# dangut/RGBiD-SLAM

Measured on AMD Instinct MI355X. Metric: aligned RGB-D frames/sec @640x480, 3-level pyr; achieved HBM GB/s vs roofline, higher is better.
Workload: dtype f32

## Files before the change

include/rgbid_batched.h:

```cpp
#ifndef RGBID_BATCHED_H_
#define RGBID_BATCHED_H_

#include "rgbid.h"

#ifdef __cplusplus
extern "C" {
#endif

typedef struct rgbid_imgb {
  void*  data;
  size_t step;
  size_t lane_stride;
  int    rows, cols;
} rgbid_imgb;

typedef struct rgbid_sys_params {
  float sigma_depthinv, sigma_int, bias_depthinv, bias_int, nu_depthinv, nu_int;
  int mestimator, weighting;
  int student_nu;
  int nu_int_from_max;
} rgbid_sys_params;

enum {
  RGBID_WM_AUTO = -1,
// ... 15 lines not shown
                            const rgbid_imgb* dst_iD, const rgbid_imgb* dst_I, const float* R_proj, const float* t_proj,
                            int numerics, float* ms);

int rgbid_lattice_pack_batched(rgbid_ctx*, int lanes, const rgbid_imgb* W0, const rgbid_imgb* I0, int min_nsamples, float* out_dev,
                               size_t out_lane_stride, float* ms);
int rgbid_lattice_residuals_batched(rgbid_ctx*, int lanes, const rgbid_imgb* Wcur, const rgbid_imgb* W0, const rgbid_imgb* Icur,
                                    const rgbid_imgb* I0, const float* R_proj, const float* t_proj, int min_nsamples, int numerics,
                                    const float* kf_lat_dev, size_t kf_lat_lane_stride, float* res_dev, size_t res_lane_stride,
                                    float* ms);
int rgbid_lattice_residuals_raw_batched(rgbid_ctx*, int lanes, const rgbid_imgb* Wcur, const rgbid_imgb* W0, const rgbid_imgb* Icur,
                                        const rgbid_imgb* I0, const float* R_proj, const float* t_proj, int min_nsamples, int numerics,
                                        const float* kf_lat_dev, size_t kf_lat_lane_stride, float* res_dev, size_t res_lane_stride,
                                        const rgbid_imgb* depth_u16, const rgbid_imgb* rgb_u8x3, float factor_depth, const int* lane_on_dev,
                                        float* ms);
int rgbid_frame_px_batched(rgbid_ctx*, int lanes, const rgbid_imgb* depth_u16, const rgbid_imgb* rgb_u8x3, const rgbid_imgb* depthinv,
                           const rgbid_imgb* intensity_pair, const rgbid_imgb* intensity_single, float factor_depth, float* ms);
typedef struct rgbid_scale_pair { float bias_depthinv, sigma_depthinv, nu_depthinv, bias_int, sigma_int, nu_int; } rgbid_scale_pair;
int rgbid_sigma_pair_batched(rgbid_ctx*, int lanes, const float* res_dev, size_t res_lane_stride, int n, int mestimator,
                             rgbid_scale_pair* out, float* ms);
int rgbid_sigma_pair_maps_batched(rgbid_ctx*, int lanes, const rgbid_imgb* W1, const rgbid_imgb* W0, const rgbid_imgb* I1, const rgbid_imgb* I0,
                                  int min_nsamples, int mestimator, rgbid_scale_pair* out, float* ms);

int rgbid_fuse_frame_batched(rgbid_ctx*, int lanes, const rgbid_imgb* cur_depthinv, const rgbid_imgb* kf_depthinv,
                             const rgbid_imgb* kf_weight, const rgbid_imgb* warped_weight, const float* R_proj, const float* t_proj,
                             int numerics, float* ms);
int rgbid_kf_maps_batched(rgbid_ctx*, int lanes, rgbid_intr intr, const rgbid_imgb* depthinv, const rgbid_imgb* vmap,
                          const rgbid_imgb* nmap, float* ms);
int rgbid_visibility_pair_batched(rgbid_ctx*, int lanes, const rgbid_imgb* a, const rgbid_imgb* b, const float* R_ab, const float* t_ab,
                                  const float* R_ba, const float* t_ba, int numerics, unsigned int* counts, float* ms);

int rgbid_prep_frame_batched(rgbid_ctx*, int lanes, const rgbid_imgb* depth_u16, const rgbid_imgb* rgb_u8x3, const rgbid_imgb* depthinv,
                             const rgbid_imgb* intensity, const rgbid_imgb* r, const rgbid_imgb* g, const rgbid_imgb* b,
                             float factor_depth, float* ms);
int rgbid_pyr_down_batched(rgbid_ctx*, int lanes, const rgbid_imgb* src, const rgbid_imgb* dst, float* ms);
int rgbid_compute_gradient_batched(rgbid_ctx*, int lanes, const rgbid_imgb* src, const rgbid_imgb* dst_hor, const rgbid_imgb* dst_vert,
                                   float* ms);
int rgbid_gradient_keep_batched(rgbid_ctx*, int lanes, const rgbid_imgb* src, const rgbid_imgb* dst_hor, const rgbid_imgb* dst_vert,
                                const rgbid_imgb* keep, float* ms);
int rgbid_bilateral_filter_batched(rgbid_ctx*, int lanes, const rgbid_imgb* src, const rgbid_imgb* dst, float sigma_floatmap,
                                   int numerics, float* ms);
int rgbid_pyr_down_pair_batched(rgbid_ctx*, int lanes, const rgbid_imgb* src0, const rgbid_imgb* dst0, const rgbid_imgb* src1,
                                const rgbid_imgb* dst1, float* ms);
int rgbid_gradient_pair_batched(rgbid_ctx*, int lanes, const rgbid_imgb* src0, const rgbid_imgb* dst_hor0, const rgbid_imgb* dst_vert0,
                                const rgbid_imgb* src1, const rgbid_imgb* dst_hor1, const rgbid_imgb* dst_vert1, float* ms);
int rgbid_gradient_keep_pair_batched(rgbid_ctx*, int lanes, const rgbid_imgb* src0, const rgbid_imgb* dst_hor0, const rgbid_imgb* dst_vert0,
                                     const rgbid_imgb* keep0, const rgbid_imgb* src1, const rgbid_imgb* dst_hor1,
                                     const rgbid_imgb* dst_vert1, const rgbid_imgb* keep1, float* ms);
int rgbid_bilateral_pair_batched(rgbid_ctx*, int lanes, const rgbid_imgb* src0, const rgbid_imgb* dst0, float sigma_floatmap0,
                                 const rgbid_imgb* src1, const rgbid_imgb* dst1, float sigma_floatmap1, int numerics, float* ms);

#ifdef __cplusplus
}
#endif
#endif
```

rgbid-slam_amd/csrc/c_api_batched.hip:

```cpp
#include "../../include/rgbid_batched.h"
#include "hip_host.h"
#include "kernels.h"

#include <cstring>
#include <vector>

using namespace rgbid;

namespace {

const LaneMask ALL{nullptr, 0};

inline bool ok_b(const rgbid_imgb* i, int lanes, size_t elem = 4) {
  const size_t align = elem == 3 ? 1 : elem;
  return i && i->data && lanes >= 1 && lanes <= 65535 && i->rows > 0 && i->cols > 0 && i->step >= (size_t)i->cols * elem && i->step % align == 0 &&
         ((uintptr_t)i->data) % align == 0 && i->rows < (1 << 24) && i->step < ((size_t)1 << 24) && (unsigned long long)i->rows * i->step < (1ull << 32) &&
         (lanes == 1 || (i->lane_stride >= (size_t)i->rows * i->step && i->lane_stride % align == 0));
}
inline bool same_b(const rgbid_imgb* a, const rgbid_imgb* b) { return a->rows == b->rows && a->cols == b->cols; }
inline ImgB BB(const rgbid_imgb* i, int lanes) { return ImgB{i->data, i->step, lanes == 1 ? 0 : i->lane_stride, i->rows, i->cols}; }
inline bool numerics_ok(int n) { return n == RGBID_NUMERICS_EXACT || n == RGBID_NUMERICS_FAST; }
inline bool al16(const rgbid_imgb* a, int lanes) { return (a->step & 15) == 0 && (lanes == 1 || (a->lane_stride & 15) == 0) && (((uintptr_t)a->data) & 15) == 0; }

struct Call {
// ... 305 lines not shown
  const size_t off_ab = 0, off_ba = up256(sizeof(WarpParams) * lanes), off_cnt = off_ba + up256(sizeof(WarpParams) * lanes);
  int e = ctx_reserve_lane(c, off_cnt + sizeof(unsigned int) * 4 * lanes);
  if (e) return e;
  if ((e = staging_free(c))) return e;
  if ((e = stage_warps(c, lanes, R_ab, t_ab, off_ab))) return e;
  if ((e = stage_warps(c, lanes, R_ba, t_ba, off_ba))) return e;
  if ((e = staging_sent(c))) return e;
  unsigned int* cnt = reinterpret_cast<unsigned int*>((char*)c->lane_dev + off_cnt);
  RGBID_HIP(hipMemsetAsync(cnt, 0, sizeof(unsigned int) * 4 * lanes, c->stream));
  Call call(c, ms);
  launch_visibility_pair(c->stream, lanes, BB(a, lanes), BB(b, lanes), reinterpret_cast<const WarpParams*>((char*)c->lane_dev + off_ab),
                         reinterpret_cast<const WarpParams*>((char*)c->lane_dev + off_ba), cnt, cnt + 2 * lanes, ALL, numerics == RGBID_NUMERICS_FAST);
  e = call.finish(cnt, sizeof(unsigned int) * 4 * lanes, off_cnt);
  if (e) return e;
  const unsigned int* h = reinterpret_cast<const unsigned int*>((char*)c->lane_host + off_cnt);
  for (int l = 0; l < lanes; ++l) {
    counts[4 * l + 0] = h[2 * l + 0]; counts[4 * l + 1] = h[2 * l + 1];
    counts[4 * l + 2] = h[2 * lanes + 2 * l + 0]; counts[4 * l + 3] = h[2 * lanes + 2 * l + 1];
  }
  return RGBID_OK;
}

int rgbid_prep_frame_batched(rgbid_ctx* c, int lanes, const rgbid_imgb* depth, const rgbid_imgb* rgb, const rgbid_imgb* iD, const rgbid_imgb* I, const rgbid_imgb* r,
                             const rgbid_imgb* g, const rgbid_imgb* b, float factor_depth, float* ms) {
  const rgbid_imgb* all[7] = {depth, rgb, iD, I, r, g, b};
  if (!c || lanes < 1 || !(factor_depth == factor_depth) || factor_depth == 0.f) return RGBID_E_INVALID;
  for (int i = 0; i < 7; ++i) if (!ok_b(all[i], lanes, i == 0 ? 2 : i == 1 ? 3 : 4) || !same_b(all[i], iD)) return RGBID_E_INVALID;
  hipSetDevice(c->device);
  Call call(c, ms);
  launch_prep_frame(c->stream, lanes, BB(depth, lanes), BB(rgb, lanes), BB(iD, lanes), BB(I, lanes), BB(r, lanes), BB(g, lanes), BB(b, lanes), factor_depth, ALL);
  return call.finish();
}

int rgbid_pyr_down_batched(rgbid_ctx* c, int lanes, const rgbid_imgb* src, const rgbid_imgb* dst, float* ms) {
  if (!c || lanes < 1 || !ok_b(src, lanes) || !ok_b(dst, lanes) || dst->rows != src->rows / 2 || dst->cols != src->cols / 2) return RGBID_E_INVALID;
  hipSetDevice(c->device);
  Call call(c, ms);
  launch_pyr_down(c->stream, lanes, BB(src, lanes), BB(dst, lanes), ALL);
  return call.finish();
}

int rgbid_compute_gradient_batched(rgbid_ctx* c, int lanes, const rgbid_imgb* src, const rgbid_imgb* gx, const rgbid_imgb* gy, float* ms) {
  if (!c || lanes < 1 || !ok_b(src, lanes) || !ok_b(gx, lanes) || !ok_b(gy, lanes) || !same_b(src, gx) || !same_b(src, gy)) return RGBID_E_INVALID;
  hipSetDevice(c->device);
  Call call(c, ms);
  launch_gradient(c->stream, lanes, BB(src, lanes), BB(gx, lanes), BB(gy, lanes), ALL);
  return call.finish();
}

int rgbid_gradient_keep_batched(rgbid_ctx* c, int lanes, const rgbid_imgb* src, const rgbid_imgb* gx, const rgbid_imgb* gy, const rgbid_imgb* keep, float* ms) {
  if (!c || lanes < 1 || !ok_b(src, lanes) || !ok_b(gx, lanes) || !ok_b(gy, lanes) || !ok_b(keep, lanes) || !same_b(src, gx) || !same_b(src, gy) || !same_b(src, keep) ||
      src->data == keep->data)
    return RGBID_E_INVALID;
  hipSetDevice(c->device);
  Call call(c, ms);
  const bool launched = launch_gradient_keep(c->stream, lanes, BB(src, lanes), BB(gx, lanes), BB(gy, lanes), BB(keep, lanes), ALL);
  const int r = call.finish();
  return launched ? r : RGBID_E_INVALID;
}

int rgbid_bilateral_filter_batched(rgbid_ctx* c, int lanes, const rgbid_imgb* src, const rgbid_imgb* dst, float sigma_floatmap, int numerics, float* ms) {
  if (!c || lanes < 1 || !ok_b(src, lanes) || !ok_b(dst, lanes) || !same_b(src, dst) || src->data == dst->data || !numerics_ok(numerics) ||
      !(sigma_floatmap > 0.f))
    return RGBID_E_INVALID;
  hipSetDevice(c->device);
  Call call(c, ms);
// ... 54 lines not shown
```

rgbid-slam_amd/csrc/engine.hip:

```cpp
#include "../../include/rgbid_engine.h"
#include "hip_host.h"
#include "kernels.h"
#include "../../include/rgbid/se3.h"
#include "engine_device.h"
#include "step_plan.h"
#include "sigma_device.h"

#include <algorithm>
#include <cassert>
#include <cstdio>
#include <cstdlib>
#include <cstring>
#include <new>
#include <vector>

#pragma clang fp contract(off)

using namespace rgbid;
using namespace rgbid::eng;

constexpr int MAXL = 8;

namespace {

// ... 131 lines not shown
  __shared__ WarpParams next_warp;
  __shared__ int update_ok;
  reduce_partials<256>(partials, nblk, lane, tid, sm, sums);
  if (tid == 0) {
    LaneState& s = st[lane];
    GnUpdate u;
    gn_update(sums, pin ? s.alt_R : s.cur_R, pin ? s.alt_t : s.cur_t, u);
    if (!u.failed) set_warp_from_pose(c, level, u.R, u.t, next_warp);
    update_ok = u.failed ? 0 : 1;
    if (blockIdx.x == 0) gn_commit(u, s, pin ? s.cur_R : s.alt_R, pin ? s.cur_t : s.alt_t, f, wp, &next_warp, c, level, lane);
  }
  __syncthreads();
  if (!update_ok) return;
  const int i = blockIdx.x * 256 + tid;
  if (i >= n) return;
  FusedLatticeGetter g{Wcur, Icur, W0, I0, next_warp, lane, stride, interp_mode, fast};
  const int ly = i / lcols, lx = i - ly * lcols;
  float rd, ri;
  if (kf_lat) {
    const float* k = kf_lat + (size_t)lane * kf_lat_lane_stride;
    g.both_given(ly, lx, k[i], k[n + i], rd, ri);
  } else {
    g.both(ly, lx, rd, ri);
  }
  float* r = res + (size_t)lane * res_lane_stride;
  r[i] = rd; r[n + i] = ri;
}
inline int update_prologue_max_lanes() {
  const char* e = getenv("RGBID_ENGINE_UPDATE_PROLOGUE_LANES");
  return e ? atoi(e) : 8;
}
inline bool lattice_raw_enabled() {
  const char* e = getenv("RGBID_ENGINE_LATTICE_RAW");
  return !(e && atoi(e) == 0);
}
inline int scalar_block_threads(int B) { return B > 256 ? 64 : 256; }

__global__ void k_level_begin(Flags f, int B) {
  int lane = blockIdx.x * blockDim.x + threadIdx.x;
  if (lane < B) f.lvl[lane] = f.gn[lane];
}
__global__ __launch_bounds__(64) RGBID_SCALAR_KERNEL void k_chi_decide(LaneState* st, Flags f, const float* chi_out, WarpParams* wp, StepCfg c, int iter, int after_level, int B) {
  int lane = blockIdx.x * blockDim.x + threadIdx.x;
  if (lane >= B || !f.lvl[lane]) return;
  LaneState& s = st[lane];
  const float RMSE = sqrtf(chi_out[3 * lane + 0]) / sqrtf(chi_out[3 * lane + 2]);
  if (iter != 1 && RMSE > s.rmse_prev) {
    double d[3], tmp[3];
    for (int i = 0; i < 3; ++i) d[i] = s.cur_t[i] - s.inc_t[i];
    se3::m3_mulv(s.inc_inv_R, d, tmp);
    for (int i = 0; i < 3; ++i) s.cur_t[i] = tmp[i];
    se3::m3_mul(s.inc_inv_R, s.cur_R, s.cur_R);
    f.lvl[lane] = 0;
    set_warp_from_pose(c, after_level, s.cur_R, s.cur_t, wp[lane]);
    return;
  }
  s.rmse_prev = RMSE;
}

template <int NT>
__global__ __launch_bounds__(NT) RGBID_SCALAR_KERNEL void k_frame_finish(const double* partials, int nblk, LaneState* st, Flags f, const SysParams* sp,
                                                      WarpParams* vis_ab, WarpParams* vis_ba, WarpParams* ivis_ab, WarpParams* ivis_ba,
                                                      rgbid_pose_record* rec, StepCfg c) {
  int lane = blockIdx.x;
  if (!f.track[lane]) return;
  __shared__ double sm[8][32];
// ... 398 lines not shown
  Ledger led;
  auto fast_at = [&](int level) {
    return c.fast_numerics != 0 && gn_fast_supported(e->iD_kf[level], e->I_kf[level], e->gxD[level], e->gyD[level], e->gxI[level], e->gyI[level], e->I_curr[level]);
  };
  auto warp_pair = [&](int l, LaneMask m) {
    if (!(fast_at(l) && launch_warp_pair_fast(s, B, e->iD_curr[l], e->I_curr[l], e->iD_kf[l], e->wiD[l], e->wI[l], nullptr, e->wp, c.interp_mode, m)))
      launch_warp_pair(s, B, e->iD_curr[l], e->I_curr[l], e->iD_kf[l], e->wiD[l], e->wI[l], e->wp, c.interp_mode, m);
    led.add(1, 0, 20 * npx(e->iD_kf[l]));
  };
  auto chi_lattice = [&](int l, LaneMask m, double bytes) {
    int n, lr, lc, st;
    lattice_geometry(e->wI[l].rows, e->wI[l].cols, 9999999, &n, &lr, &lc, &st);
    launch_error_lattice(s, B, e->wI[l], e->I_kf[l], e->res_I, res_stride, lr, lc, st, m);
    launch_error_lattice(s, B, e->wiD[l], e->iD_kf[l], e->res_D, res_stride, lr, lc, st, m);
    launch_chi_square(s, B, e->res_I, e->res_D, res_stride, n, 5.f, 0.0025f, c.mestimator, e->chi_out, m);
    led.add(3, 0, bytes);
  };
  auto kf_maps = [&](LaneMask m, int bucket, double fallback_bytes) {
    const int n = enqueue_kf_maps(e, s, m);
    led.add(n, bucket, n == 1 ? 28 * N0 : fallback_bytes);
  };
  auto system_events = [&](int level) {
    if (!(e->prof_on && level == 0 && e->prof_used + 2 <= (int)e->prof_ev.size())) return;
    set_system_kernel_events(e->prof_ev[e->prof_used], e->prof_ev[e->prof_used + 1]);
    e->prof_used += 2;
  };
  auto per_lane = [&](auto* k64, auto* k256, auto... args) {
    const int nt = scalar_block_threads(B);
    hipLaunchKernelGGL(nt == 64 ? k64 : k256, dim3(B), dim3(nt), 0, s, args...);
    led.add(1);
  };
  const LaneMask fed = M(e->active_dev);
  const bool custom = c.custom_registration != 0;
  launch_prep_frame(s, B, e->cur_depth, e->cur_rgb, custom ? e->iD_dist : e->iD_curr[0], custom ? e->I_dist : e->I_curr[0], e->r_curr, e->g_curr, e->b_curr, c.factor_depth, fed);
  led.add(1, 0, 25 * N0);
  if (custom) {
    const IntrK kc{c.fx, c.fy, c.cx, c.cy, c.rgb_dist[0], c.rgb_dist[1], c.rgb_dist[2], c.rgb_dist[3], c.rgb_dist[4]};
    const IntrK kd{c.depth_intr.fx, c.depth_intr.fy, c.depth_intr.cx, c.depth_intr.cy, c.depth_intr.k1, c.depth_intr.k2, c.depth_intr.k3, c.depth_intr.k4, c.depth_intr.k5};
    DepthDistP dp;
    dp.c1 = c.depth_dist.c1; dp.c0 = c.depth_dist.c0; dp.xshift = c.depth_dist.xshift; dp.yshift = c.depth_dist.yshift;
    for (int i = 0; i < 9; ++i) { dp.q0[i] = c.depth_dist.q0[i]; dp.q1[i] = c.depth_dist.q1[i]; }
    launch_undistort(s, B, e->I_dist, e->I_curr[0], kc, true, c.interp_mode, fed);
    led.add(1, 0, 12 * N0);
    launch_depthinv_correction(s, B, e->iD_dist, e->iD_corr, kd, dp, fed);
    led.add(1, 0, 8 * N0);
    launch_undistort(s, B, e->iD_corr, e->iD_prereg, kd, false, 0, fed);
    led.add(1, 0, 8 * N0);
    launch_register_depthinv(s, B, e->iD_prereg, e->reg_f, e->reg_i, e->iD_curr[0], c.dRc_proj, c.t_dc_proj, c.cRd_proj, fed);
    led.add(4, 0, (9 * 4 + 8 + 9 * 8 + 8) * N0);
  }
  for (int i = 1; i < L; ++i) {
    launch_pyr_down2(s, B, e->I_curr[i - 1], e->I_curr[i], e->iD_curr[i - 1], e->iD_curr[i], fed);
    led.add(1, 0, 2 * (4 * npx(e->I_curr[i - 1]) + 4 * npx(e->I_curr[i])));
  }
  hipLaunchKernelGGL(k_step_begin, dim3(gb), dim3(tb), 0, s, e->state, f, e->wp, e->sp, sc, B, e->counts, e->sched.start_sys_level, e->sched.start_sys_cov);
  led.add(1);
  if (!first) {
    const bool chi_stop = c.termination == RGBID_CHI_SQUARED, warp_first = c.warping == RGBID_WARP_FIRST, pdf = c.sigma_estimator == RGBID_SIGMA_PDF;
    const LaneMask LV = M(f.lvl), GN = M(f.gn);
    assert(!(c.fused_gn && (warp_first || chi_stop)));
    const bool prologue_plan = c.fused_gn && pdf && e->lat_res && B <= update_prologue_max_lanes();
    const RawFrame raw0{e->cur_depth, e->cur_rgb, c.factor_depth};
    const bool lattice_raw = lattice_raw_enabled() && !custom && !prologue_plan && fast_at(0) && lattice_raw_supported(raw0, e->iD_kf[0], B);
    struct { bool on; int nblk, sys_level, sys_cov; } pend = {false, 0, -1, 0};
    int pose_in_alt = 0;
    int nblk;
    for (const GnIter& g : e->sched.iters) {
      const int level = g.level;
      if (chi_stop && g.it == 0) { hipLaunchKernelGGL(k_level_begin, dim3(gb), dim3(tb), 0, s, f, B); led.add(1); }
      const double nl = npx(e->iD_kf[level]);
      const double ns = pdf ? (double)lattice_samples(e->iD_kf[level].rows, e->iD_kf[level].cols, c.nsamples) : 0.0;
      if (c.fused_gn) {
        if (pdf) {
          if (pend.on) {
            int n_, lr_, lc_, st_;
            lattice_geometry(e->iD_kf[level].rows, e->iD_kf[level].cols, c.nsamples, &n_, &lr_, &lc_, &st_);
            const size_t kls = 2 * e->lat_cap;
            hipLaunchKernelGGL(k_lattice_after_update, dim3(div_up(n_, 256), B), dim3(256), 0, s, e->iD_curr[level], e->iD_kf[level], e->I_curr[level], e->I_kf[level], c.interp_mode,
                               n_, lc_, st_, e->lat_res, 2 * e->lat_cap, kls >= 2 * (size_t)n_ ? e->lat_kf[level] : nullptr, kls, fast_at(level) ? 1 : 0,
                               e->partials, pend.nblk, e->state, f, e->wp, sc, level, e->sp, pend.sys_level, pend.sys_cov, pose_in_alt);
            launch_sigma_pair_arrays(s, B, e->lat_res, 2 * e->lat_cap, n_, e->sp, c.mestimator, LV);
            pose_in_alt ^= 1; pend.on = false;
          } else {
            launch_sigma_pair_fused(s, B, e->iD_curr[level], e->iD_kf[level], e->I_curr[level], e->I_kf[level], e->wp, c.interp_mode, c.nsamples,
// ... 508 lines not shown
```

rgbid-slam_amd/csrc/kernels.h:

```cpp
#pragma once
#include "common.h"

namespace rgbid {

struct SysParams {
  float fx, fy, cx, cy;
  float sigma_d, sigma_i, bias_d, bias_i, nu_d, nu_i;
  int mestimator, weighting, student_nu;
  int nu_i_max;
};
struct SigmaIO { float bias, sigma, nu; };
struct IntrP { float fx, fy, cx, cy; };
struct LightP { float x, y, z; };
struct IntrK { float fx, fy, cx, cy, k1, k2, k3, k4, k5; };
struct DepthDistP { float c1, c0, q0[9], q1[9]; int xshift, yshift; };

enum { SYS_TERMS = 27 };
static constexpr float TH_HUBER = 1.345f, TH_TUKEY = 4.685f, STUDENT_DOF = 5.f;

void launch_undistort(hipStream_t s, int B, ImgB src, ImgB dst, IntrK k, bool linear, int interp_mode, LaneMask m);
void launch_depthinv_correction(hipStream_t s, int B, ImgB src, ImgB dst, IntrK k, DepthDistP dp, LaneMask m);
void launch_register_depthinv(hipStream_t s, int B, ImgB src, ImgB inter_f, ImgB inter_i, ImgB dst, const float dRc_proj[9], const float t_dc_proj[3],
                              const float cRd_proj[9], LaneMask m);

void launch_depth_to_invdepth(hipStream_t s, int B, ImgB src_u16, ImgB dst, float factor_depth, LaneMask m);
void launch_intensity(hipStream_t s, int B, ImgB rgb, ImgB dst, LaneMask m);
void launch_depth_to_float(hipStream_t s, int B, ImgB src_u16, ImgB dst, LaneMask m);
void launch_float_to_rgb(hipStream_t s, int B, ImgB src, ImgB dst_rgb, LaneMask m);
void launch_warp_pair(hipStream_t s, int B, ImgB src_iD, ImgB src_I, ImgB grid, ImgB dst_iD, ImgB dst_I, const WarpParams* lane_params, int interp_mode, LaneMask m,
                      const WarpParams* host_p = nullptr);
bool launch_warp_pair_fast(hipStream_t s, int B, ImgB src_iD, ImgB src_I, ImgB grid, ImgB dst_iD, ImgB dst_I, const WarpParams* host_p, const WarpParams* lane_params,
                           int interp_mode, LaneMask m);
void launch_selftest_cvt_flr(hipStream_t s, unsigned long long* mismatches_dev, unsigned stride);
void launch_nmap_cross(hipStream_t s, int B, ImgB vmap, ImgB nmap, LaneMask m);
void launch_integrate_warped_rgb(hipStream_t s, int B, ImgB warped, ImgB r, ImgB g, ImgB b, ImgB wweight, ImgB kf, ImgB colors, ImgB kfw, LaneMask m);
void launch_decompose_rgb(hipStream_t s, int B, ImgB rgb, ImgB r, ImgB g, ImgB b, LaneMask m);
void launch_gradient(hipStream_t s, int B, ImgB src, ImgB gx, ImgB gy, LaneMask m);
bool launch_gradient_keep(hipStream_t s, int B, ImgB src, ImgB gx, ImgB gy, ImgB keep, LaneMask m);
void launch_prep_frame(hipStream_t s, int B, ImgB depth_u16, ImgB rgb, ImgB iD, ImgB I, ImgB r, ImgB g, ImgB b, float factor_depth, LaneMask m);
void launch_copy_bytes(hipStream_t s, int B, ImgB src, ImgB dst, int elem_size, LaneMask m);
void launch_fill(hipStream_t s, int B, ImgB dst, int elem_size, uint32_t bits, LaneMask m);
void launch_pyr_down(hipStream_t s, int B, ImgB src, ImgB dst, LaneMask m);
void launch_pyr_down2(hipStream_t s, int B, ImgB src0, ImgB dst0, ImgB src1, ImgB dst1, LaneMask m);
void launch_gradient2(hipStream_t s, int B, ImgB src0, ImgB gx0, ImgB gy0, ImgB src1, ImgB gx1, ImgB gy1, LaneMask m);
bool launch_gradient_keep2(hipStream_t s, int B, ImgB src0, ImgB gx0, ImgB gy0, ImgB keep0, ImgB src1, ImgB gx1, ImgB gy1, ImgB keep1, LaneMask m);
void launch_bilateral2(hipStream_t s, int B, ImgB src0, ImgB dst0, float sigma0, ImgB src1, ImgB dst1, float sigma1, LaneMask m, bool fast = false);
void launch_lattice_pack_levels(hipStream_t s, int B, int n_levels, const ImgB* W0, const ImgB* I0, int min_nsamples, float* const* out, size_t out_lane_stride, LaneMask m);
void launch_visibility_pair2(hipStream_t s, int B, ImgB a, ImgB b0, const WarpParams* p_ab0, const WarpParams* p_ba0, unsigned int* counts_ab0, unsigned int* counts_ba0,
                             ImgB b1, const WarpParams* p_ab1, const WarpParams* p_ba1, unsigned int* counts_ab1, unsigned int* counts_ba1, LaneMask m, bool fast);
void launch_bilateral(hipStream_t s, int B, ImgB src, ImgB dst, float sigma_floatmap, LaneMask m, bool fast = false);
bool div_const_verified(float c);
void launch_selftest_div_const(hipStream_t s, float c, unsigned long long* mismatches_dev);

void launch_warp_invdepth(hipStream_t s, int B, ImgB src, ImgB grid, ImgB dst, const WarpParams* host_p, const WarpParams* lane_p, LaneMask m);
void launch_warp_intensity(hipStream_t s, int B, ImgB src, ImgB grid, ImgB dst, const WarpParams* host_p, const WarpParams* lane_p, int interp_mode, LaneMask m);
void launch_warp_invdepth_weighted(hipStream_t s, int B, ImgB src, ImgB grid, ImgB dst, ImgB weight, const WarpParams* host_p, const WarpParams* lane_p, LaneMask m);
void launch_integrate_warped(hipStream_t s, int B, ImgB warped, ImgB wweight, ImgB kf, ImgB kfweight, LaneMask m);
void launch_visibility(hipStream_t s, int B, ImgB src, ImgB dst, ImgB mask, const WarpParams* host_p, const WarpParams* lane_p, unsigned int* counts, LaneMask m);
void launch_visibility_pair(hipStream_t s, int B, ImgB a, ImgB b, const WarpParams* p_ab, const WarpParams* p_ba, unsigned int* counts_ab,
                            unsigned int* counts_ba, LaneMask m, bool fast = false);
void launch_vmap(hipStream_t s, int B, ImgB depthinv, ImgB vmap, IntrP k, LaneMask m);
void launch_nmap_gradients(hipStream_t s, int B, ImgB depthinv, ImgB gx, ImgB gy, ImgB nmap, IntrP k, LaneMask m);
bool launch_fuse_frame(hipStream_t s, int B, ImgB src, ImgB kf, ImgB kfw, ImgB wweight, const WarpParams* lane_params, LaneMask m, bool fast = false);
bool launch_kf_maps(hipStream_t s, int B, ImgB depthinv, ImgB vmap, ImgB nmap, IntrP k, LaneMask m);
void launch_generate_image(hipStream_t s, int B, ImgB vmap, ImgB nmap, ImgB rgb, ImgB dst, const LightP* host_l, const LightP* lane_l, LaneMask m);

struct RawFrame { ImgB depth, rgb; float factor_depth; };
void lattice_geometry(int rows, int cols, int min_nsamples, int* n, int* lrows, int* lcols, int* stride);
void launch_error_lattice(hipStream_t s, int B, ImgB im1, ImgB im0, float* err, size_t err_lane_stride, int lrows, int lcols, int stride, LaneMask m);
void launch_sigma(hipStream_t s, int B, int mode, const float* err, size_t err_lane_stride, int n, SigmaIO* io, int mestimator, LaneMask m);
void launch_sigma_pair(hipStream_t s, int B, ImgB W1, ImgB W0, ImgB I1, ImgB I0, int min_nsamples, SysParams* sp, int mestimator, LaneMask m);
void launch_sigma_pair_fused(hipStream_t s, int B, ImgB Wcur, ImgB W0, ImgB Icur, ImgB I0, const WarpParams* lane_wp, int interp_mode,
// ... 25 lines not shown
```

rgbid-slam_amd/csrc/kernels_prep.hip:

```cpp
#include "kernels.h"
#include "warp_device.h"

#pragma clang fp contract(off)

namespace rgbid {

static constexpr int TX = 64, TY = 4;
static constexpr int RPB = 16;

static inline dim3 grid2d(int cols, int rows, int B) { return dim3(div_up(cols, TX), div_up(rows, TY * RPB), B); }
#define RGBID_FOR_TILES(y0v) for (int it_ = 0, y0v = blockIdx.y * (TY * RPB); it_ < RPB; ++it_, y0v += TY)

__global__ __launch_bounds__(256) void k_depth_to_invdepth(ImgB src, ImgB dst, float factor_depth, LaneMask m) {
  int lane = blockIdx.z;
  if (!m.on(lane)) return;
  int x = blockIdx.x * TX + threadIdx.x;
  RGBID_FOR_TILES(y0) {
    int y = y0 + threadIdx.y;
    if (x >= dst.cols || y >= dst.rows) continue;
    int value = px<uint16_t>(src, lane, y, x);
    float r = qnan();
    if (value > 0) r = (1.f / factor_depth) * 1000.f / (float)max(0, min(value, 10000));
    px<float>(dst, lane, y, x) = r;
  }
// ... 395 lines not shown
#pragma unroll
          for (int dx = 0; dx < 5; ++dx) sum1 = sum1 + win[2 * j + dy].v[dx] * W.w[(dx - 2) * (dx - 2) + (dy - 2) * (dy - 2)];
        if (writer) px<float>(dst, lane, y, x) = sum1 / W.sum_all;
        continue;
      }
      float sum1 = 0.f, sum2 = 0.f, count = 0.f;
#pragma unroll
      for (int dy = 0; dy < 5; ++dy)
#pragma unroll
        for (int dx = 0; dx < 5; ++dx) {
          const float weight = W.w[(dx - 2) * (dx - 2) + (dy - 2) * (dy - 2)];
          sum1 = sum1 + win[2 * j + dy].v[dx] * weight;
          sum2 = __builtin_fmaf(win[2 * j + dy].m[dx], weight, sum2);
          count += win[2 * j + dy].m[dx];
        }
      if (writer) px<float>(dst, lane, y, x) = count > 12.f ? sum1 / sum2 : qnan();
    }
  }
}
void launch_pyr_down(hipStream_t s, int B, ImgB src, ImgB dst, LaneMask m) {
  int strips = div_up(dst.rows, PD_ROWS);
  const int wpr = div_up(dst.cols, PD_WAVE_OUT);
  const int wgs = div_up(strips * wpr, 4);
  hipLaunchKernelGGL(k_pyr_down_dpp, dim3((unsigned)wgs * (unsigned)B), dim3(256), 0, s, src, dst, src, dst, pyr_weights(), strips, wpr, wgs, wgs * B, m);
}
void launch_pyr_down2(hipStream_t s, int B, ImgB src0, ImgB dst0, ImgB src1, ImgB dst1, LaneMask m) {
  if (!(same_geometry(src0, src1) && same_geometry(dst0, dst1))) { launch_pyr_down(s, B, src0, dst0, m); launch_pyr_down(s, B, src1, dst1, m); return; }
  int strips = div_up(dst0.rows, PD_ROWS);
  const int wpr = div_up(dst0.cols, PD_WAVE_OUT);
  const int wgs = div_up(strips * wpr, 4);
  hipLaunchKernelGGL(k_pyr_down_dpp, dim3(2u * (unsigned)wgs * (unsigned)B), dim3(256), 0, s, src0, dst0, src1, dst1, pyr_weights(), strips, wpr, wgs, wgs * B, m);
}

__global__ __launch_bounds__(256) void k_selftest_div_const(DivConst d, unsigned long long* mismatches) {
  const uint32_t hi = blockIdx.x;
  unsigned int bad = 0;
  for (uint32_t lo = threadIdx.x; lo < 65536u; lo += blockDim.x) {
    const float x = __uint_as_float((hi << 16) | lo);
    bool ok;
    const float a = div_const_fast(x, d, ok), b = x / d.c;
    const bool same = (__float_as_uint(a) == __float_as_uint(b)) || (a == 0.f && b == 0.f);
    bad += (ok && !same) ? 1u : 0u;
  }
  if (bad) atomicAdd(mismatches, (unsigned long long)bad);
}
void launch_selftest_div_const(hipStream_t s, float c, unsigned long long* mismatches_dev) {
  hipLaunchKernelGGL(k_selftest_div_const, dim3(65536), dim3(256), 0, s, DivConst{c, 1.0f / c}, mismatches_dev);
}

}
```

rgbid-slam_amd/rgbid/batched.py:

```python
import ctypes as C

import numpy as np
import torch

from . import _lib
from ._lib import Intr, check

NUMERICS_EXACT, NUMERICS_FAST = 0, 1
WM_AUTO, WM_GENERIC, WM_STUDENT_NU, WM_STUDENT_FIXED = -1, 0, 1, 2

BATCHED_EXPORTS = [
    "rgbid_gn_fused_batched", "rgbid_build_system_batched", "rgbid_warp_pair_batched", "rgbid_lattice_pack_batched",
    "rgbid_lattice_residuals_batched", "rgbid_sigma_pair_batched", "rgbid_fuse_frame_batched", "rgbid_kf_maps_batched",
    "rgbid_visibility_pair_batched", "rgbid_prep_frame_batched", "rgbid_pyr_down_batched", "rgbid_compute_gradient_batched",
    "rgbid_bilateral_filter_batched", "rgbid_gradient_keep_batched", "rgbid_lattice_residuals_raw_batched", "rgbid_frame_px_batched",
    "rgbid_sigma_pair_maps_batched", "rgbid_pyr_down_pair_batched", "rgbid_gradient_pair_batched", "rgbid_gradient_keep_pair_batched",
    "rgbid_bilateral_pair_batched",
]


class ImgB(C.Structure):
    _fields_ = [("data", C.c_void_p), ("step", C.c_size_t), ("lane_stride", C.c_size_t), ("rows", C.c_int), ("cols", C.c_int)]


class SysParams(C.Structure):
    _fields_ = [("sigma_depthinv", C.c_float), ("sigma_int", C.c_float), ("bias_depthinv", C.c_float), ("bias_int", C.c_float),
                ("nu_depthinv", C.c_float), ("nu_int", C.c_float), ("mestimator", C.c_int), ("weighting", C.c_int),
                ("student_nu", C.c_int), ("nu_int_from_max", C.c_int)]


class ScalePair(C.Structure):
    _fields_ = [(n, C.c_float) for n in ("bias_depthinv", "sigma_depthinv", "nu_depthinv", "bias_int", "sigma_int", "nu_int")]


def imgb(t):
    if not t.is_cuda:
        raise _lib.RgbidError("rgbid images must live in device memory (no CPU path)")
    es = t.element_size()
    if t.dim() == 4:
        assert t.shape[3] == 3 and t.dtype == torch.uint8 and t.stride(3) == 1 and t.stride(2) == 3
    else:
        assert t.dim() == 3 and t.stride(2) == 1
    return ImgB(t.data_ptr(), t.stride(1) * es, t.stride(0) * es, t.shape[1], t.shape[2])


def _f32(a, lanes, n):
    a = np.ascontiguousarray(np.asarray(a, np.float32).reshape(lanes, n))
    return a, a.ctypes.data_as(C.c_void_p)


# ... 94 lines not shown
                                                   C.byref(ms)))
        return [dict(bias_depthinv=o.bias_depthinv, sigma_depthinv=o.sigma_depthinv, nu_depthinv=o.nu_depthinv, bias_int=o.bias_int,
                     sigma_int=o.sigma_int, nu_int=o.nu_int) for o in out]

    def fuse_frame(self, cur_iD, kf_iD, kf_weight, warped_weight, R_proj, t_proj, fast=False):
        lanes = kf_iD.shape[0]
        Rk, Rp = _f32(R_proj, lanes, 9); tk, tp = _f32(t_proj, lanes, 3)
        ms = C.c_float()
        check(self.L.rgbid_fuse_frame_batched(self._h, lanes, *[C.byref(imgb(t)) for t in (cur_iD, kf_iD, kf_weight, warped_weight)], Rp, tp,
                                              int(bool(fast)), C.byref(ms)))
        return ms.value

    def kf_maps(self, intr, depthinv, vmap, nmap):
        lanes = depthinv.shape[0]
        ms = C.c_float()
        check(self.L.rgbid_kf_maps_batched(self._h, lanes, Intr(*intr), C.byref(imgb(depthinv)), C.byref(imgb(vmap)), C.byref(imgb(nmap)), C.byref(ms)))
        return ms.value

    def visibility_pair(self, a, b, R_ab, t_ab, R_ba, t_ba, fast=False):
        lanes = a.shape[0]
        k1, p1 = _f32(R_ab, lanes, 9); k2, p2 = _f32(t_ab, lanes, 3); k3, p3 = _f32(R_ba, lanes, 9); k4, p4 = _f32(t_ba, lanes, 3)
        counts = np.zeros((lanes, 4), np.uint32); ms = C.c_float()
        check(self.L.rgbid_visibility_pair_batched(self._h, lanes, C.byref(imgb(a)), C.byref(imgb(b)), p1, p2, p3, p4, int(bool(fast)),
                                                   counts.ctypes.data_as(C.c_void_p), C.byref(ms)))
        return counts

    def prep_frame(self, depth_u16, rgb, iD, I, r, g, b, factor_depth=1.0):
        lanes = iD.shape[0]
        ms = C.c_float()
        check(self.L.rgbid_prep_frame_batched(self._h, lanes, *[C.byref(imgb(t)) for t in (depth_u16, rgb, iD, I, r, g, b)], C.c_float(factor_depth),
                                              C.byref(ms)))
        return ms.value

    def pyr_down(self, src, dst):
        ms = C.c_float()
        check(self.L.rgbid_pyr_down_batched(self._h, src.shape[0], C.byref(imgb(src)), C.byref(imgb(dst)), C.byref(ms)))
        return ms.value

    def gradient(self, src, gx, gy):
        ms = C.c_float()
        check(self.L.rgbid_compute_gradient_batched(self._h, src.shape[0], C.byref(imgb(src)), C.byref(imgb(gx)), C.byref(imgb(gy)), C.byref(ms)))
        return ms.value

    def gradient_keep(self, src, gx, gy, keep):
        ms = C.c_float()
        check(self.L.rgbid_gradient_keep_batched(self._h, src.shape[0], C.byref(imgb(src)), C.byref(imgb(gx)), C.byref(imgb(gy)), C.byref(imgb(keep)), C.byref(ms)))
        return ms.value

    def bilateral(self, src, dst, sigma_floatmap, fast=False):
        ms = C.c_float()
        check(self.L.rgbid_bilateral_filter_batched(self._h, src.shape[0], C.byref(imgb(src)), C.byref(imgb(dst)), C.c_float(sigma_floatmap),
                                                    int(bool(fast)), C.byref(ms)))
        return ms.value

    def pyr_down_pair(self, src0, dst0, src1, dst1):
        ms = C.c_float()
        check(self.L.rgbid_pyr_down_pair_batched(self._h, src0.shape[0], *[C.byref(imgb(t)) for t in (src0, dst0, src1, dst1)], C.byref(ms)))
        return ms.value

    def gradient_pair(self, src0, gx0, gy0, src1, gx1, gy1):
        ms = C.c_float()
        check(self.L.rgbid_gradient_pair_batched(self._h, src0.shape[0], *[C.byref(imgb(t)) for t in (src0, gx0, gy0, src1, gx1, gy1)], C.byref(ms)))
        return ms.value

    def gradient_keep_pair(self, src0, gx0, gy0, keep0, src1, gx1, gy1, keep1):
        ms = C.c_float()
# ... 10 lines not shown
```

Measured before the change: 27460.

## Fuse frame prep with first pyramid downsample into one DPP kernel

Adds a kernel that converts raw u16 depth and u8 RGB into inverse depth, intensity and colour planes while computing the level-1 pyramid in the same pass. Level-0 planes are written and also kept in registers for the 5x5 Gaussian. This removes a separate pyr_down launch and its re-read of the level-0 maps from HBM. The cost is a more complex, register-heavy kernel. It is only used when no custom registration is configured and the vector alignment and geometry checks pass, with an env var to disable it.

```diff
diff --git a/include/rgbid_batched.h b/include/rgbid_batched.h
--- a/include/rgbid_batched.h
+++ b/include/rgbid_batched.h
@@ -71,6 +71,9 @@
 int rgbid_prep_frame_batched(rgbid_ctx*, int lanes, const rgbid_imgb* depth_u16, const rgbid_imgb* rgb_u8x3, const rgbid_imgb* depthinv,
                              const rgbid_imgb* intensity, const rgbid_imgb* r, const rgbid_imgb* g, const rgbid_imgb* b,
                              float factor_depth, float* ms);
+int rgbid_prep_frame_pyr_batched(rgbid_ctx*, int lanes, const rgbid_imgb* depth_u16, const rgbid_imgb* rgb_u8x3, const rgbid_imgb* depthinv,
+                                 const rgbid_imgb* intensity, const rgbid_imgb* r, const rgbid_imgb* g, const rgbid_imgb* b,
+                                 const rgbid_imgb* depthinv1, const rgbid_imgb* intensity1, float factor_depth, float* ms);
 int rgbid_pyr_down_batched(rgbid_ctx*, int lanes, const rgbid_imgb* src, const rgbid_imgb* dst, float* ms);
 int rgbid_compute_gradient_batched(rgbid_ctx*, int lanes, const rgbid_imgb* src, const rgbid_imgb* dst_hor, const rgbid_imgb* dst_vert,
                                    float* ms);
diff --git a/rgbid-slam_amd/csrc/c_api_batched.hip b/rgbid-slam_amd/csrc/c_api_batched.hip
--- a/rgbid-slam_amd/csrc/c_api_batched.hip
+++ b/rgbid-slam_amd/csrc/c_api_batched.hip
@@ -361,6 +361,20 @@
   return call.finish();
 }
 
+int rgbid_prep_frame_pyr_batched(rgbid_ctx* c, int lanes, const rgbid_imgb* depth, const rgbid_imgb* rgb, const rgbid_imgb* iD, const rgbid_imgb* I, const rgbid_imgb* r,
+                                 const rgbid_imgb* g, const rgbid_imgb* b, const rgbid_imgb* iD1, const rgbid_imgb* I1, float factor_depth, float* ms) {
+  const rgbid_imgb* all[7] = {depth, rgb, iD, I, r, g, b};
+  if (!c || lanes < 1 || !(factor_depth == factor_depth) || factor_depth == 0.f) return RGBID_E_INVALID;
+  for (int i = 0; i < 7; ++i) if (!ok_b(all[i], lanes, i == 0 ? 2 : i == 1 ? 3 : 4) || !same_b(all[i], iD)) return RGBID_E_INVALID;
+  if (!ok_b(iD1, lanes) || !ok_b(I1, lanes) || !same_b(iD1, I1)) return RGBID_E_INVALID;
+  hipSetDevice(c->device);
+  Call call(c, ms);
+  const bool launched = launch_prep_frame_pyr(c->stream, lanes, BB(depth, lanes), BB(rgb, lanes), BB(iD, lanes), BB(I, lanes), BB(r, lanes), BB(g, lanes), BB(b, lanes),
+                                              BB(iD1, lanes), BB(I1, lanes), factor_depth, ALL);
+  const int e = call.finish();
+  return launched ? e : RGBID_E_INVALID;
+}
+
 int rgbid_pyr_down_batched(rgbid_ctx* c, int lanes, const rgbid_imgb* src, const rgbid_imgb* dst, float* ms) {
   if (!c || lanes < 1 || !ok_b(src, lanes) || !ok_b(dst, lanes) || dst->rows != src->rows / 2 || dst->cols != src->cols / 2) return RGBID_E_INVALID;
   hipSetDevice(c->device);
diff --git a/rgbid-slam_amd/csrc/engine.hip b/rgbid-slam_amd/csrc/engine.hip
--- a/rgbid-slam_amd/csrc/engine.hip
+++ b/rgbid-slam_amd/csrc/engine.hip
@@ -187,6 +187,10 @@
 }
 inline bool lattice_raw_enabled() {
   const char* e = getenv("RGBID_ENGINE_LATTICE_RAW");
+  return !(e && atoi(e) == 0);
+}
+inline bool prep_pyr_enabled() {
+  const char* e = getenv("RGBID_ENGINE_PREP_PYR");
   return !(e && atoi(e) == 0);
 }
 inline int scalar_block_threads(int B) { return B > 256 ? 64 : 256; }
@@ -651,8 +655,14 @@
   };
   const LaneMask fed = M(e->active_dev);
   const bool custom = c.custom_registration != 0;
-  launch_prep_frame(s, B, e->cur_depth, e->cur_rgb, custom ? e->iD_dist : e->iD_curr[0], custom ? e->I_dist : e->I_curr[0], e->r_curr, e->g_curr, e->b_curr, c.factor_depth, fed);
-  led.add(1, 0, 25 * N0);
+  const bool prep_pyr = !custom && L > 1 && prep_pyr_enabled() &&
+                        launch_prep_frame_pyr(s, B, e->cur_depth, e->cur_rgb, e->iD_curr[0], e->I_curr[0], e->r_curr, e->g_curr, e->b_curr, e->iD_curr[1], e->I_curr[1], c.factor_depth, fed);
+  if (prep_pyr) {
+    led.add(2, 0, 25 * N0 + 2 * (4 * npx(e->I_curr[0]) + 4 * npx(e->I_curr[1])));
+  } else {
+    launch_prep_frame(s, B, e->cur_depth, e->cur_rgb, custom ? e->iD_dist : e->iD_curr[0], custom ? e->I_dist : e->I_curr[0], e->r_curr, e->g_curr, e->b_curr, c.factor_depth, fed);
+    led.add(1, 0, 25 * N0);
+  }
   if (custom) {
     const IntrK kc{c.fx, c.fy, c.cx, c.cy, c.rgb_dist[0], c.rgb_dist[1], c.rgb_dist[2], c.rgb_dist[3], c.rgb_dist[4]};
     const IntrK kd{c.depth_intr.fx, c.depth_intr.fy, c.depth_intr.cx, c.depth_intr.cy, c.depth_intr.k1, c.depth_intr.k2, c.depth_intr.k3, c.depth_intr.k4, c.depth_intr.k5};
@@ -668,7 +678,7 @@
     launch_register_depthinv(s, B, e->iD_prereg, e->reg_f, e->reg_i, e->iD_curr[0], c.dRc_proj, c.t_dc_proj, c.cRd_proj, fed);
     led.add(4, 0, (9 * 4 + 8 + 9 * 8 + 8) * N0);
   }
-  for (int i = 1; i < L; ++i) {
+  for (int i = prep_pyr ? 2 : 1; i < L; ++i) {
     launch_pyr_down2(s, B, e->I_curr[i - 1], e->I_curr[i], e->iD_curr[i - 1], e->iD_curr[i], fed);
     led.add(1, 0, 2 * (4 * npx(e->I_curr[i - 1]) + 4 * npx(e->I_curr[i])));
   }
diff --git a/rgbid-slam_amd/csrc/kernels.h b/rgbid-slam_amd/csrc/kernels.h
--- a/rgbid-slam_amd/csrc/kernels.h
+++ b/rgbid-slam_amd/csrc/kernels.h
@@ -38,6 +38,7 @@
 void launch_gradient(hipStream_t s, int B, ImgB src, ImgB gx, ImgB gy, LaneMask m);
 bool launch_gradient_keep(hipStream_t s, int B, ImgB src, ImgB gx, ImgB gy, ImgB keep, LaneMask m);
 void launch_prep_frame(hipStream_t s, int B, ImgB depth_u16, ImgB rgb, ImgB iD, ImgB I, ImgB r, ImgB g, ImgB b, float factor_depth, LaneMask m);
+bool launch_prep_frame_pyr(hipStream_t s, int B, ImgB depth_u16, ImgB rgb, ImgB iD, ImgB I, ImgB r, ImgB g, ImgB b, ImgB iD1, ImgB I1, float factor_depth, LaneMask m);
 void launch_copy_bytes(hipStream_t s, int B, ImgB src, ImgB dst, int elem_size, LaneMask m);
 void launch_fill(hipStream_t s, int B, ImgB dst, int elem_size, uint32_t bits, LaneMask m);
 void launch_pyr_down(hipStream_t s, int B, ImgB src, ImgB dst, LaneMask m);
diff --git a/rgbid-slam_amd/csrc/kernels_prep.hip b/rgbid-slam_amd/csrc/kernels_prep.hip
--- a/rgbid-slam_amd/csrc/kernels_prep.hip
+++ b/rgbid-slam_amd/csrc/kernels_prep.hip
@@ -451,6 +451,170 @@
   hipLaunchKernelGGL(k_pyr_down_dpp, dim3(2u * (unsigned)wgs * (unsigned)B), dim3(256), 0, s, src0, dst0, src1, dst1, pyr_weights(), strips, wpr, wgs, wgs * B, m);
 }
 
+struct PrepPyrFrame { ImgB depth, rgb, iD, I, r, g, b; };
+struct PrepPx { float2 w, R, G, B; };
+template <bool COLOUR>
+__device__ __forceinline__ uint2 prep_issue_pair(__amdgpu_buffer_rsrc_t rs, unsigned pitch_b, int rows, int cy, unsigned colb) {
+  const unsigned rb = __umul24((unsigned)((cy >= 0 && cy < rows) ? cy : 0), pitch_b);
+  if (COLOUR) return __builtin_bit_cast(uint2, __builtin_amdgcn_raw_buffer_load_b64(rs, rb + colb, 0, 0));
+  return uint2{__builtin_bit_cast(unsigned, __builtin_amdgcn_raw_buffer_load_b32(rs, rb + colb, 0, 0)), 0u};
+}
+template <bool COLOUR>
+__device__ __forceinline__ PrepPx prep_convert_pair(uint2 q, unsigned sh, float scale) {
+  PrepPx o;
+  if (COLOUR) {
+    const unsigned lo = __builtin_amdgcn_alignbyte(q.y, q.x, sh), hi = __builtin_amdgcn_alignbyte(0u, q.y, sh);
+    const unsigned r0 = lo & 255u, g0 = (lo >> 8) & 255u, b0 = (lo >> 16) & 255u, r1 = lo >> 24, g1 = hi & 255u, b1 = (hi >> 8) & 255u;
+    o.w = float2{frame_px(0u, r0, g0, b0, 0.f).I, frame_px(0u, r1, g1, b1, 0.f).I};
+    o.R = float2{(float)r0, (float)r1}; o.G = float2{(float)g0, (float)g1}; o.B = float2{(float)b0, (float)b1};
+  } else {
+    o.w = float2{frame_px(q.x & 0xffffu, 0u, 0u, 0u, scale).iD, frame_px(q.x >> 16, 0u, 0u, 0u, scale).iD};
+    o.R = o.G = o.B = float2{0.f, 0.f};
+  }
+  return o;
+}
+struct PrepQuad { float a, b, c, d; };
+__device__ __forceinline__ PrepQuad prep_gather4(float2 o, float2 e, bool odd) {
+  const float e0 = dpp_shift<0x138>(e.x), e1 = dpp_shift<0x138>(e.y), o2 = dpp_shift<0x130>(o.x), o3 = dpp_shift<0x130>(o.y);
+  return PrepQuad{odd ? o.x : e0, odd ? o.y : e1, odd ? o2 : e.x, odd ? o3 : e.y};
+}
+#ifndef RGBID_PREP_PYR_STORE_AUX
+#define RGBID_PREP_PYR_STORE_AUX 2
+#endif
+struct PrepPlane {
+  __amdgpu_buffer_rsrc_t rsrc;
+  unsigned pitch_b;
+  typedef float f4v __attribute__((ext_vector_type(4)));
+  typedef int v4i __attribute__((ext_vector_type(4)));
+  __device__ __forceinline__ PrepPlane(const ImgB& im, int lane)
+      : rsrc(__builtin_amdgcn_make_buffer_rsrc(row_ptr<float>(im, lane, 0), 0, (int)((unsigned)im.rows * (unsigned)im.pitch), 0x00020000)), pitch_b((unsigned)im.pitch) {}
+  __device__ __forceinline__ void st16_stream(int y, unsigned voff, const PrepQuad& q) const {
+    __builtin_amdgcn_raw_buffer_store_b128(__builtin_bit_cast(v4i, f4v{q.a, q.b, q.c, q.d}), rsrc, voff, (unsigned)y * pitch_b, RGBID_PREP_PYR_STORE_AUX);
+  }
+};
+__device__ __forceinline__ void prep_store_rows(const PrepPlane& P, int y, unsigned voff, float2 top, float2 bot, bool odd, bool writer, bool has_bot) {
+  const PrepQuad q = prep_gather4(bot, top, odd);
+  if (writer && (!odd || has_bot)) P.st16_stream(y, voff + (odd ? P.pitch_b : 0u), q);
+}
+template <bool COLOUR>
+__device__ __forceinline__ void prep_pyr_walk(const PrepPyrFrame& F, const ImgB& dst, float factor_depth, const PyrWeights& W, int lane, int strip, int wx, int lid) {
+  const ImgB& src = COLOUR ? F.I : F.iD;
+  const ImgB& raw = COLOUR ? F.rgb : F.depth;
+  const int x = wx * PD_WAVE_OUT + lid - 1;
+  const int y_begin = strip * PD_ROWS;
+  const bool c0 = x >= 0 && 2 * x < src.cols, c1 = x >= 0 && 2 * x + 1 < src.cols;
+  const bool writer = lid >= 1 && lid <= PD_WAVE_OUT && x < dst.cols;
+  const bool odd = (lid & 1) != 0;
+  const float scale = frame_depth_scale(factor_depth);
+  const __amdgpu_buffer_rsrc_t rs = __builtin_amdgcn_make_buffer_rsrc(row_ptr<uint8_t>(raw, lane, 0), 0,
+      (int)((unsigned)(raw.rows - 1) * (unsigned)raw.pitch + (COLOUR ? 3u : 2u) * (unsigned)raw.cols), 0x00020000);
+  const unsigned pitch_b = (unsigned)raw.pitch;
+  const unsigned xb = (unsigned)max(x, 0);
+  const unsigned colb = COLOUR ? (6u * xb) & ~3u : 4u * xb;
+  const unsigned sh = COLOUR ? (6u * xb) & 2u : 0u;
+  const unsigned voff = (unsigned)(2 * x - (odd ? 0 : 2)) << 2;
+  const PrepPlane pW(src, lane), pR(F.r, lane), pG(F.g, lane), pB(F.b, lane);
+  auto store_rows = [&](const PrepPx& top, const PrepPx& bot, int cy, bool has_bot) {
+    prep_store_rows(pW, cy, voff, top.w, bot.w, odd, writer, has_bot);
+    if (COLOUR) {
+      prep_store_rows(pR, cy, voff, top.R, bot.R, odd, writer, has_bot);
+      prep_store_rows(pG, cy, voff, top.G, bot.G, odd, writer, has_bot);
+      prep_store_rows(pB, cy, voff, top.B, bot.B, odd, writer, has_bot);
+    }
+  };
+  const float mc2 = c0 ? 1.f : 0.f, mc3 = c1 ? 1.f : 0.f;
+  const float mc[5] = {dpp_shift<0x138>(mc2), dpp_shift<0x138>(mc3), mc2, mc3, dpp_shift<0x130>(mc2)};
+  PyrRow win[2 * PD_ROWS + 3];
+  bool full[2 * PD_ROWS + 3], rin[2 * PD_ROWS + 3];
+  uint2 rawv[2 * PD_ROWS + 3];
+  auto finish = [&](float2 p, int r, bool row_in) {
+    rin[r] = row_in;
+    if (COLOUR) {
+      PyrRow& o = win[r];
+      const float v0 = (row_in && c0) ? p.x : 0.f, v1 = (row_in && c1) ? p.y : 0.f;
+      o.v[2] = v0; o.v[3] = v1; o.v[0] = dpp_shift<0x138>(v0); o.v[1] = dpp_shift<0x138>(v1); o.v[4] = dpp_shift<0x130>(v0);
+      full[r] = __ballot(row_in && c0 && c1) == ~0ull;
+    } else {
+      full[r] = pyr_finish_shared(p, row_in, c0, c1, win[r]);
+    }
+  };
+#pragma unroll
+  for (int r = 0; r < 3 + 2 * PD_AHEAD; ++r) rawv[r] = prep_issue_pair<COLOUR>(rs, pitch_b, src.rows, 2 * y_begin - 2 + r, colb);
+#pragma unroll
+  for (int r = 0; r < 3; ++r) {
+    const int cy = 2 * y_begin - 2 + r;
+    const PrepPx c = prep_convert_pair<COLOUR>(rawv[r], sh, scale);
+    if (r == 2 && y_begin == 0) store_rows(c, c, 0, false);
+    finish(c.w, r, cy >= 0 && cy < src.rows);
+  }
+#pragma unroll
+  for (int j = 0; j < PD_ROWS; ++j) {
+    const int y = y_begin + j;
+    if (y < dst.rows) {
+      if (j + PD_AHEAD < PD_ROWS && y + PD_AHEAD < dst.rows) {
+        rawv[2 * (j + PD_AHEAD) + 3] = prep_issue_pair<COLOUR>(rs, pitch_b, src.rows, 2 * (y + PD_AHEAD) + 1, colb);
+        rawv[2 * (j + PD_AHEAD) + 4] = prep_issue_pair<COLOUR>(rs, pitch_b, src.rows, 2 * (y + PD_AHEAD) + 2, colb);
+      }
+      const PrepPx ca = prep_convert_pair<COLOUR>(rawv[2 * j + 3], sh, scale), cb = prep_convert_pair<COLOUR>(rawv[2 * j + 4], sh, scale);
+      store_rows(ca, cb, 2 * y + 1, 2 * y + 2 < src.rows);
+      const float2 wa = ca.w, wb = cb.w;
+      __builtin_amdgcn_sched_barrier(0);
+      finish(wa, 2 * j + 3, 2 * y + 1 < src.rows);
+      finish(wb, 2 * j + 4, 2 * y + 2 < src.rows);
+      if (W.sum_all > 0.f && full[2 * j] && full[2 * j + 1] && full[2 * j + 2] && full[2 * j + 3] && full[2 * j + 4]) {
+        float sum1 = 0.f;
+#pragma unroll
+        for (int dy = 0; dy < 5; ++dy)
+#pragma unroll
+          for (int dx = 0; dx < 5; ++dx) sum1 = sum1 + win[2 * j + dy].v[dx] * W.w[(dx - 2) * (dx - 2) + (dy - 2) * (dy - 2)];
+        if (writer) px<float>(dst, lane, y, x) = sum1 / W.sum_all;
+        continue;
+      }
+      float sum1 = 0.f, sum2 = 0.f, count = 0.f;
+#pragma unroll
+      for (int dy = 0; dy < 5; ++dy) {
+        if (COLOUR && !rin[2 * j + dy]) continue;
+#pragma unroll
+        for (int dx = 0; dx < 5; ++dx) {
+          const float weight = W.w[(dx - 2) * (dx - 2) + (dy - 2) * (dy - 2)];
+          const float mask = COLOUR ? mc[dx] : win[2 * j + dy].m[dx];
+          sum1 = sum1 + win[2 * j + dy].v[dx] * weight;
+          sum2 = __builtin_fmaf(mask, weight, sum2);
+          count += mask;
+        }
+      }
+      if (writer) px<float>(dst, lane, y, x) = count > 12.f ? sum1 / sum2 : qnan();
+    }
+  }
+}
+__global__ __launch_bounds__(256) void k_prep_pyr_dpp(PrepPyrFrame F, ImgB iD1, ImgB I1, float factor_depth, PyrWeights W, int strips, int wpr, int wgs_per_lane, LaneMask m) {
+  const unsigned V = xcd_slab_index(blockIdx.x, gridDim.x);
+  const unsigned half_lane = V / (unsigned)wgs_per_lane;
+  const int wg = (int)(V - half_lane * (unsigned)wgs_per_lane), lane = (int)(half_lane >> 1);
+  const bool depth_half = (half_lane & 1u) != 0;
+  if (!m.on(lane)) return;
+  const int wave = __builtin_amdgcn_readfirstlane((wg * 256 + (int)threadIdx.x) >> 6), lid = threadIdx.x & 63;
+  if (wave >= strips * wpr) return;
+  const int strip = wave / wpr, wx = wave - strip * wpr;
+  if (depth_half) prep_pyr_walk<false>(F, iD1, factor_depth, W, lane, strip, wx, lid);
+  else prep_pyr_walk<true>(F, I1, factor_depth, W, lane, strip, wx, lid);
+}
+bool launch_prep_frame_pyr(hipStream_t s, int B, ImgB depth, ImgB rgb, ImgB iD, ImgB I, ImgB r, ImgB g, ImgB b, ImgB iD1, ImgB I1, float factor_depth, LaneMask m) {
+  const bool vec = (iD.cols % 4 == 0) && vec4_ok(iD, 4) && vec4_ok(I, 4) && vec4_ok(r, 4) && vec4_ok(g, 4) && vec4_ok(b, 4) &&
+                   ((depth.pitch & 7) == 0) && ((depth.lane_stride & 7) == 0) && ((((uintptr_t)depth.base) & 7) == 0) &&
+                   ((rgb.pitch & 3) == 0) && ((rgb.lane_stride & 3) == 0) && ((((uintptr_t)rgb.base) & 3) == 0);
+  const bool geo = same_geometry(iD, I) && same_geometry(iD, r) && same_geometry(iD, g) && same_geometry(iD, b) && same_geometry(iD, depth) && same_geometry(iD, rgb) &&
+                   same_geometry(iD1, I1) && iD1.rows >= 1 && iD1.cols >= 1 && iD.rows == 2 * iD1.rows && iD.cols == 2 * iD1.cols;
+  auto small = [](const ImgB& a) { return a.pitch < ((size_t)1 << 24) && (unsigned long long)a.rows * a.pitch < (1ull << 31); };
+  if (!(vec && geo && small(depth) && small(rgb) && small(iD) && small(I) && small(r) && small(g) && small(b) && small(iD1) && small(I1) &&
+        depth.pitch >= 2 * (size_t)depth.cols && rgb.pitch >= 3 * (size_t)rgb.cols))
+    return false;
+  const int strips = div_up(iD1.rows, PD_ROWS), wpr = div_up(iD1.cols, PD_WAVE_OUT), wgs = div_up(strips * wpr, 4);
+  hipLaunchKernelGGL(k_prep_pyr_dpp, dim3(2u * (unsigned)wgs * (unsigned)B), dim3(256), 0, s, PrepPyrFrame{depth, rgb, iD, I, r, g, b}, iD1, I1, factor_depth,
+                     pyr_weights(), strips, wpr, wgs, m);
+  return true;
+}
+
 __global__ __launch_bounds__(256) void k_selftest_div_const(DivConst d, unsigned long long* mismatches) {
   const uint32_t hi = blockIdx.x;
   unsigned int bad = 0;
diff --git a/rgbid-slam_amd/rgbid/batched.py b/rgbid-slam_amd/rgbid/batched.py
--- a/rgbid-slam_amd/rgbid/batched.py
+++ b/rgbid-slam_amd/rgbid/batched.py
@@ -15,7 +15,7 @@
     "rgbid_visibility_pair_batched", "rgbid_prep_frame_batched", "rgbid_pyr_down_batched", "rgbid_compute_gradient_batched",
     "rgbid_bilateral_filter_batched", "rgbid_gradient_keep_batched", "rgbid_lattice_residuals_raw_batched", "rgbid_frame_px_batched",
     "rgbid_sigma_pair_maps_batched", "rgbid_pyr_down_pair_batched", "rgbid_gradient_pair_batched", "rgbid_gradient_keep_pair_batched",
-    "rgbid_bilateral_pair_batched",
+    "rgbid_bilateral_pair_batched", "rgbid_prep_frame_pyr_batched",
 ]
 
 
@@ -176,6 +176,13 @@
                                               C.byref(ms)))
         return ms.value
 
+    def prep_frame_pyr(self, depth_u16, rgb, iD, I, r, g, b, iD1, I1, factor_depth=1.0):
+        lanes = iD.shape[0]
+        ms = C.c_float()
+        check(self.L.rgbid_prep_frame_pyr_batched(self._h, lanes, *[C.byref(imgb(t)) for t in (depth_u16, rgb, iD, I, r, g, b, iD1, I1)],
+                                                  C.c_float(factor_depth), C.byref(ms)))
+        return ms.value
+
     def pyr_down(self, src, dst):
         ms = C.c_float()
         check(self.L.rgbid_pyr_down_batched(self._h, src.shape[0], C.byref(imgb(src)), C.byref(imgb(dst)), C.byref(ms)))
```

New measurement: 27650, median of 4. No clear change (+0.7%).
